# potsawee/tokenize-audio

Hardware: AMD Instinct MI355X
Metric: audio-sec encoded/sec (Mimi 8-codebook, 24 kHz) (higher is better)
Workload: dtype f16x3 (fp32-emulating: 2 fp16 planes per operand, 3 products, fp32 accumulate; RVQ distances fp32); 1 GPU; LibriTTS-R-style batch encode (configs[1]): batch=32 x 10 s @ 24 kHz resident in HBM, K=8 codebooks, 1 encode per step per GPU; global_batch=32, num_quantizers=8, parallelism=utterance round-robin x1 (no collective), gemm_precision=f16x3

## Files before the change

### tokenize-audio_amd/csrc/engine.cpp

```cpp
#include <hip/hip_runtime.h>

#include <algorithm>
#include <cmath>
#include <cstdarg>
#include <cstdio>
#include <cstdlib>
#include <cstring>
#include <fstream>
#include <map>
#include <memory>
#include <mutex>
#include <string>
#include <tuple>
#include <unordered_map>
#include <vector>

#include "../../include/mimi_hip.h"
#include "host_io.h"
#include "kernels.h"

using namespace mimi;

static thread_local std::string g_last_error;

// ... 267 lines not shown
    int stage0_fused = 1;
    int ln_fused = 1;
    int rvq_form = 0;
    int ln_rpw = 1;
    int rvq_xcd = 1;
    int rvq_chain = 1;
    bool chain_ok = false;
    unsigned* chain_flag = nullptr;
    int rvq_chain_fault = 0;
    int64_t chain_reruns = 0;
    int qkv_attn = 1;
    int qkv_attn_xcd = 1;
    int attn_band_split = 1;
    int sc1_out = 2;
    int fc1_cg = 1;
    int res1_form = 1;
    int res1_stream = 1;
    struct Tap {
        float* d = nullptr;
        size_t cap = 0;
        int64_t dims[3] = {0, 0, 0};
    };
    std::map<std::string, Tap> tapmap;

    bool decode_enabled = false;
    DevConv dec_first, dec_last;
    std::vector<DevConv> dec_up;
    std::vector<DevConv> dec_res3, dec_res1;
    std::vector<DevXfmr> dxf;
    float* outproj = nullptr;
// ... 1117 lines not shown
                ad.C = nullptr;
                xact = new_act("x_last");
                out_act(ad, xact);
            } else if (next_unf) {
                ad.Cp = w.xe;
                ad.c_pstride = (long long)B * p.T[si + 1] * 2 * C;
                role = ROLE_DOWN_XE;
                xeact = new_act(nmf("xe%d", si + 1));
                out_act(ad, xeact);
            }
        }
        if (rg) {
            ad.a_rows = dT[si];
            ad.m_rows = dT[si + 1];
        }
        LAUNCH_TRY(launch_gemm(role, ad, s, &kname, prec), "down");
        snprintf(nm, sizeof nm, "down_s%d", si);
        rec.mark(nm, gemm_flops(ad) * rows_of(si + 1, (double)B * p.T[si + 1]) / ((double)B * p.T[si + 1]),
                 gemm_bytes(ad, false), kname);
        snprintf(nm, sizeof nm, last ? "down%d_elu" : "down%d", si);
        if ((rc = save_tap_planes(e, nm, w.x, last ? ns : 0, B, p.T[si + 1], 2 * C, s, last ? xact.scale : 0.0f)))
            return rc;
        C *= 2;
    }
    const int64_t T = p.frames25;
    const int Hd = c.hidden_size;
    GemmArgs af = conv_args(e->final_conv, w.x, p.T[c.num_ratios], w.t0, T, B);
    if (ns) planes_in(af, w.x, (long long)B * p.T[c.num_ratios] * C);
    use_h(af, e->final_conv.wh, e->final_conv.wscale, xact);
    if (rg) {
        af.a_rows = dT[c.num_ratios];
// ... 14 lines not shown
        double f = 0;
        for (int64_t i = 0; i < Tn; ++i) f += 4.0 * Dh * std::min<int64_t>(i + 1, c.sliding_window);
        return f * H;
    };
    if (rg) {
        for (const auto& pb : rg->plan) att_flops += att_fl(pb.frames25);
    } else {
        att_flops = att_fl(T) * B;
    }
    for (int l = 0; l < c.num_hidden_layers; ++l) {
        const DevXfmr& x = e->xf[l];
        const long long nact = rows * Hd;
        Act t1a = new_act(nmf("xf%d.ln1", l));
        if (ln_check_free(t1a, x.ln1_bound)) t1a.amax = nullptr;
        auto ln_into = [&](GemmArgs& g, int role, const float* lw, const float* lb, const Act& act) {
            if (!h16 || e->ln_fused < (role == ROLE_QKV ? 2 : 1) || !gemm_ln_prologue_ok(role, g, prec)) return false;
            if (role == ROLE_QKV) g.ln_tile = e->ln_fused - 2;
            g.ln_x = w.t0;
            g.ln_g = lw;
            g.ln_b = lb;
            g.ln_eps = c.norm_eps;
            g.ln_scale = act.scale;
            g.ln_amax = act.amax;
            return true;
        };
        GemmArgs aq = linear_args(w.t1, T, Hd, x.wqkv, 3 * H * Dh, w.qkv);
        aq.Wsplit = x.wqkv_s;
        aq.batch = B;
        aq.a_bstride = T * Hd;
        aq.c_bstride = T * 3 * H * Dh;
        aq.rope_cos = e->rope_cos;
// ... 79 lines not shown
            use_h(a1, x.w1_h, x.w1_hs, t1b);
            a1.Cp = w.ff;
            a1.c_pstride = rows * c.intermediate_size;
            a1.C = nullptr;
            ffa = new_act(nmf("xf%d.ff", l));
            out_act(a1, ffa);
        }
        if (!ln_into(a1, ROLE_FC1, x.ln2_w, x.ln2_b, t1b)) {
            LAUNCH_TRY(launch_layernorm(w.t0, x.ln2_w, x.ln2_b, w.t1, rows, Hd, c.norm_eps, s, w.t1, nact, ns, t1b.scale,
                                        t1b.amax, nullptr, 0, e->ln_rpw),
                       "ln2");
            rec.mark("layernorm", 0, 2.0 * rows * Hd * 4, ln_kname(e->ln_rpw));
        }
        a1.sc1 = (e->sc1_out & 2) != 0;
        a1.ncg = e->fc1_cg;
        LAUNCH_TRY(launch_gemm(ROLE_FC1, a1, s, &kname, prec), "fc1");
        rec.mark("fc1", gemm_flops(a1), gemm_bytes(a1, false), kname);
        if ((rc = save_tap_planes(e, nmf("ff%d", l).c_str(), w.ff, ns, tapB, tapT, c.intermediate_size, s, ffa.scale)))
            return rc;
        GemmArgs a2 = linear_args(w.ff, rows, c.intermediate_size, x.w2, Hd, w.t0);
        a2.Wsplit = x.w2_s;
        a2.R = w.t0;
        a2.scale = x.ls2;
        if (ns) planes_in(a2, w.ff, rows * (long long)c.intermediate_size);
        use_h(a2, x.w2_h, x.w2_hs, ffa);
        if (ds_planes && l == c.num_hidden_layers - 1) {
            a2.Cp = w.t1;
            a2.c_pstride = nact;
            dsin = new_act("ds.in");
            out_act(a2, dsin);
        }
// ... 1219 lines not shown
    const char* values;
};
static const EngineOption kEngineOptions[] = {
    {"stage0_fused", &mimi_engine::stage0_fused, 0x3u, "0 or 1"},
    {"rvq_form", &mimi_engine::rvq_form, 0x7fu, "0..6"},
    {"ln_rpw", &mimi_engine::ln_rpw, 0x117u, "0, 1, 2, 4 or 8"},
    {"rvq_xcd", &mimi_engine::rvq_xcd, 0x3u, "0 or 1"},
    {"rvq_chain", &mimi_engine::rvq_chain, 0x3u, "0 or 1"},
    {"rvq_chain_fault", &mimi_engine::rvq_chain_fault, 0x7u, "0, 1 or 2"},
    {"sc1_out", &mimi_engine::sc1_out, 0xffu, "0..7"},
    {"ln_fused", &mimi_engine::ln_fused, 0x1fu, "0 .. 4"},
    {"qkv_attn", &mimi_engine::qkv_attn, 0x7u, "0, 1 or 2"},
    {"qkv_attn_xcd", &mimi_engine::qkv_attn_xcd, 0x3u, "0 or 1"},
    {"attn_band_split", &mimi_engine::attn_band_split, 0x7u, "0, 1 or 2"},
    {"fc1_cg", &mimi_engine::fc1_cg, 0x17u, "0, 1, 2 or 4"},
    {"res1_form", &mimi_engine::res1_form, 0x3u, "0 or 1"},
    {"res1_stream", &mimi_engine::res1_stream, 0x7u, "0, 1 or 2"},
};

extern "C" int mimi_set_option(mimi_engine* e, const char* key, int64_t value) {
    if (!e || !key) return set_err(MIMI_ERR_INVALID_ARGUMENT, "null engine or key");
    std::lock_guard<std::mutex> lk(e->mu);
    for (const EngineOption& o : kEngineOptions) {
        if (strcmp(key, o.key)) continue;
        if (value < 0 || value > 31 || !((o.allowed >> value) & 1u))
            return set_err(MIMI_ERR_INVALID_ARGUMENT, "%s %lld (%s)", key, (long long)value, o.values);
        HIP_TRY(hipSetDevice(e->device));
        if (e->*o.field != (int)value) {
            drop_graphs(e);
            e->graph_seen.clear();
// ... 156 lines not shown
```

### tokenize-audio_amd/csrc/gemm.hip

```cpp
#include <algorithm>
#include <cstdio>
#include <cstdlib>


#include "gemm_planes.h"

#ifndef MIMI_QKV_V
#define MIMI_QKV_V 1
#endif
#ifndef MIMI_FC1_V
#define MIMI_FC1_V 0
#endif
#ifndef MIMI_SMALL16_32W
#define MIMI_SMALL16_32W 1
#endif
#ifndef MIMI_SMALL16_32
#define MIMI_SMALL16_32 15
#endif


namespace mimi {

template <int BM, int BN, int WM, int WN, int BK, int NBUF, bool NFAST, bool ELU_IN, int PAD, int EPI, int TAG>
static const char* kernel_symbol() {
// ... 61 lines not shown
    long long grid = nwg;
    if (FL & FL_PERSIST) {
        static const int slots = [kern] {
            int dev = 0, ncu = 256, occ = 1;
            (void)hipGetDevice(&dev);
            (void)hipDeviceGetAttribute(&ncu, hipDeviceAttributeMultiprocessorCount, dev);
            (void)hipOccupancyMaxActiveBlocksPerMultiprocessor(&occ, kern, (WM * WN + LW) * 64, 0);
            return std::max(8, ncu * std::max(1, occ) / 8 * 8);
        }();
        grid = std::min<long long>(nwg, slots);
    }
    hipLaunchKernelGGL(kern, dim3((unsigned)grid), dim3((WM * WN + LW) * 64), 0, s, a);
    return hipGetLastError();
}

template <int EPI, int OUTP3, int OUTP2, int TAG>
static hipError_t run_planes_big(const GemmArgs& a, hipStream_t s, int prec) {
    if (prec == PREC_F16X3) return run_planes<256, 128, 4, 2, 2, 3, EPI, OUTP2, TAG, 0, 32, 16, 0, true>(a, s);
    if (prec == PREC_BF16X6) return run_planes<256, 128, 4, 2, 3, 2, EPI, OUTP3, TAG>(a, s);
    return run_planes<256, 128, 4, 2, 2, 3, EPI, OUTP2, TAG>(a, s);
}
template <int EPI, int OUTP3, int OUTP2, int TAG>
static hipError_t run_planes_big_ld(const GemmArgs& a, hipStream_t s, int prec) {
    if (prec == PREC_F16X3) return run_planes<256, 128, 4, 2, 2, 3, EPI, OUTP2, TAG, 0, 32, 16, 0, true>(a, s);
    if (prec == PREC_BF16X6) return run_planes<256, 128, 2, 2, 3, 2, EPI, OUTP3, TAG, 4>(a, s);
    return run_planes<256, 128, 2, 2, 2, 3, EPI, OUTP2, TAG, 4>(a, s);
}
template <int EPI, int TAG>
static hipError_t run_planes_small(const GemmArgs& a, hipStream_t s, int prec) {
    if (prec == PREC_F16X3) return run_planes<128, 128, 4, 2, 2, 4, EPI, 0, TAG, 0, 32, 16, 0, true>(a, s);
// ... 12 lines not shown

template <bool ELU_IN, int PAD, int EPI, int TAG>
static hipError_t run_prec(const GemmArgs& a, hipStream_t s, int prec);

template <bool ELU_IN, int PAD, int EPI, int TAG>
static hipError_t run_auto(const GemmArgs& a, hipStream_t s) {
    if (a.N <= 32) return run<256, 32, 4, 1, 32, 1, false, ELU_IN, PAD, EPI, TAG>(a, s);
    if (a.N <= 64) return run<256, 64, 4, 1, 32, 1, false, ELU_IN, PAD, EPI, TAG>(a, s);
    if (a.M <= 1024) return run<64, 128, 1, 2, 32, 1, false, ELU_IN, PAD, EPI, TAG>(a, s);
    return run<128, 128, 2, 2, 32, 1, false, ELU_IN, PAD, EPI, TAG>(a, s);
}

static hipError_t dispatch(int role, const GemmArgs& a, hipStream_t s);

static thread_local int g_prec = PREC_F32;

template <bool ELU_IN, int PAD, int EPI, int TAG>
static hipError_t run_prec(const GemmArgs& a, hipStream_t s, int prec) {
    if (prec == PREC_BF16X6 || prec == PREC_F16X3) return run_split<128, 128, 2, 2, 3, ELU_IN, PAD, EPI, TAG>(a, s);
    if (prec == PREC_BF16X3) return run_split<128, 128, 2, 2, 2, ELU_IN, PAD, EPI, TAG>(a, s);
    return run_auto<ELU_IN, PAD, EPI, TAG>(a, s);
}

__global__ __launch_bounds__(256) void gelu_check_kernel(const float* __restrict__ in, long long n,
                                                         float* __restrict__ out) {
    for (long long i = blockIdx.x * 256LL + threadIdx.x; i < n; i += (long long)gridDim.x * 256) out[i] = gelu_fast(in[i]);
}
hipError_t launch_gelu_check(const float* in, long long n, float* out, hipStream_t st) {
    if (n <= 0) return hipSuccess;
    const long long blocks = std::min<long long>((n + 255) / 256, 4096);
    hipLaunchKernelGGL(gelu_check_kernel, dim3((unsigned)blocks), dim3(256), 0, st, in, n, out);
    return hipGetLastError();
}

hipError_t launch_gemm(int role, const GemmArgs& a, hipStream_t s, const char** kname, int precision) {
    if (a.K % 32 != 0 || a.a_cin % 4 != 0 || a.a_rs % 4 != 0 || a.M <= 0 || a.N <= 0 || a.batch <= 0)
        return hipErrorInvalidValue;
    if (a.Ap && (a.a_cin % 8 != 0 || a.a_rs % 8 != 0 || a.a_off % 8 != 0)) return hipErrorInvalidValue;
    g_last_kernel = nullptr;
    g_prec = precision;
    hipError_t e = dispatch(role, a, s);
    if (kname) *kname = g_last_kernel ? g_last_kernel : "?";
    return e;
}

static bool pair_ok(const GemmArgs& a) {
    if (a.a_cin <= 0 || a.a_cin % 64 || a.K % a.a_cin || a.a_rs % a.a_cin) return false;
    const int k = a.K / a.a_cin, st = a.a_rs / a.a_cin;
    return st > 0 && k == 2 * st && a.K % 64 == 0;
}

constexpr long long kSmallGrid = 128;
static long long tiles(const GemmArgs& a, int bm, int bn) {
    return (long long)((a.M + bm - 1) / bm) * ((a.N + bn - 1) / bn) * a.batch;
}

#ifndef MIMI_DOWN_SMALL_ST
#define MIMI_DOWN_SMALL_ST 6
#endif
#ifndef MIMI_DOWN_SMALL2_ST
#define MIMI_DOWN_SMALL2_ST 3
#endif
template <int EPI, int OUTP, int TAG>
static hipError_t run_planes_down_h16(const GemmArgs& a, hipStream_t s) {
    if (pair_ok(a) && tiles(a, 256, 128) < kSmallGrid && a.K >= 4096) {
        if (tiles(a, 64, 64) < 256)
            return run_planes<32, 32, 1, 2, 2, MIMI_DOWN_SMALL_ST, EPI, OUTP, TAG, 4, 32, 16, FL_PAIR | FL_KG2, true>(a, s);
// ... 8 lines not shown

#ifndef MIMI_SMALL_ST
#define MIMI_SMALL_ST 4
#endif
#ifndef MIMI_LNA_ST
#define MIMI_LNA_ST 4
#endif
template <int EPI, int OUTP, int TAG, int BN0, int BM1, int BN1, int WM1, int WN1, int BN2, int WN2, int ST = MIMI_SMALL_ST,
          int FL = 0, int BM0 = 64, int WN0 = 2>
static hipError_t run_small_h16(const GemmArgs& a, hipStream_t s) {
    if (tiles(a, BM0, BN0) >= 256) return run_planes<BM0, BN0, 2, WN0, 2, ST, EPI, OUTP, TAG, 4, 32, 16, FL, true>(a, s);
    if (tiles(a, BM1, BN1) >= 256) return run_planes<BM1, BN1, WM1, WN1, 2, ST, EPI, OUTP, TAG, 4, 32, 16, FL, true>(a, s);
    return run_planes<16, BN2, 1, WN2, 2, ST, EPI, OUTP, TAG, 4, 32, 16, FL, true>(a, s);
}

bool gemm_ln_prologue_ok(int role, const GemmArgs& a, int precision) {
    return precision == PREC_F16X3 && (role == ROLE_QKV || role == ROLE_FC1) && a.K == 512 && a.a_rs == 512 &&
           a.a_off == 0 && !a.a_rows && !a.m_rows && !a.a_boff && tiles(a, 128, 128) < kSmallGrid;
}

static hipError_t dispatch_planes(int role, const GemmArgs& a, hipStream_t s) {
    const int prec = g_prec;
    if (prec != PREC_BF16X6 && prec != PREC_BF16X3 && prec != PREC_F16X3) return hipErrorInvalidValue;
    if (a.ln_x) {
        if (!gemm_ln_prologue_ok(role, a, prec) || !a.ln_g || !a.ln_b || !(a.ln_scale > 0.0f)) return hipErrorInvalidValue;
        if (role == ROLE_QKV) {
            if (tiles(a, 32, 128) >= 256) return run_planes<32, 128, 2, 2, 2, MIMI_LNA_ST, EPI_ROPE, 0, 5, 4, 32, 16, FL_LNA, true>(a, s);
            if (a.ln_tile == 1) return run_planes<32, 64, 2, 1, 2, MIMI_LNA_ST, EPI_ROPE, 0, 5, 4, 32, 16, FL_LNA, true>(a, s);
            if (a.ln_tile == 2) return run_planes<16, 128, 1, 2, 2, MIMI_LNA_ST, EPI_ROPE, 0, 5, 4, 32, 16, FL_LNA, true>(a, s);
            return run_planes<16, 64, 1, 1, 2, MIMI_LNA_ST, EPI_ROPE, 0, 5, 4, 32, 16, FL_LNA, true>(a, s);
        }
        if (tiles(a, 64, 64) >= 256) return run_planes<64, 64, 2, 2, 2, MIMI_LNA_ST, EPI_GELU, 2, 7, 4, 32, 16, FL_LNA, true>(a, s);
        if (tiles(a, 32, 64) >= 256) return run_planes<32, 64, 2, 2, 2, MIMI_LNA_ST, EPI_GELU, 2, 7, 4, 32, 16, FL_LNA, true>(a, s);
        return run_planes<16, 64, 1, 2, 2, MIMI_LNA_ST, EPI_GELU, 2, 7, 4, 32, 16, FL_LNA, true>(a, s);
    }
#ifndef MIMI_SMALL_ROLES
#define MIMI_SMALL_ROLES 1
#endif
    const bool qsmall = tiles(a, 128, 128) < 256 &&
                        (((MIMI_SMALL_ROLES & 1) && (role == ROLE_DOWNSAMPLE || role == ROLE_INPROJ)) ||
                         ((MIMI_SMALL_ROLES & 2) && role == ROLE_OPROJ) || ((MIMI_SMALL_ROLES & 4) && role == ROLE_FC2) ||
                         ((MIMI_SMALL_ROLES & 8) && role == ROLE_FINAL));
    if (prec == PREC_F16X3 && (tiles(a, 128, 128) < kSmallGrid || qsmall)) {
        switch (role) {
            case ROLE_FINAL:
                if (MIMI_SMALL16_32 & 2) return run_small_h16<EPI_BIAS_OUT, 0, 4, 64, 32, 64, 2, 2, 32, MIMI_SMALL16_32W>(a, s);
                return run_small_h16<EPI_BIAS_OUT, 0, 4, 64, 32, 64, 2, 2, 64, 2>(a, s);
            case ROLE_QKV: return run_small_h16<EPI_ROPE, 0, 5, 128, 32, 128, 2, 2, 64, 1>(a, s);
            case ROLE_OPROJ:
// ... 108 lines not shown
```

### tokenize-audio_amd/csrc/gemm_planes.h

```cpp
#pragma once
#include <type_traits>

#include "gemm_kernel.h"

namespace mimi {

#if defined(__HIP_DEVICE_COMPILE__)
__device__ __forceinline__ __amdgpu_buffer_rsrc_t make_rsrc(const void* base, long long bytes) {
    const long long lim = bytes < 0x7fffffffLL ? bytes : 0x7fffffffLL;
    return __builtin_amdgcn_make_buffer_rsrc(const_cast<void*>(base), (short)0, (int)lim, 0x00020000);
}
#endif

template <int PM, int L>
__device__ __forceinline__ void wait_stages(int later) {
    if constexpr (L == 0) {
        asm volatile("s_waitcnt vmcnt(0)" ::: "memory");
    } else {
        if (later >= L)
            asm volatile("s_waitcnt vmcnt(%0)" ::"n"(L * PM) : "memory");
        else
            wait_stages<PM, L - 1>(later);
    }
}
// ... 39 lines not shown
    constexpr int TPA = LNA ? 0 : NS * AR / RPP, TP = TPA + NS * NB * BN / RPP;
    constexpr int PMAX = (TP + NLD - 1) / NLD;
    constexpr int PMIN = TP / NLD;
    static_assert(BK == 32 || (BK == 16 && MF == 32), "BK");
    static_assert(MF == 32 || MF == 16, "MFMA shape");
    static_assert(TM >= 1 && TN >= 1 && KSUB >= 1, "tile");
    static_assert(NS * BM % RPP == 0 && NS * BN % RPP == 0, "whole pieces");
    static_assert(STAGES >= 2 * KG && STAGES <= 16, "stages");
    static_assert(PMAX * (STAGES - 2 * KG) <= 63, "vmcnt range");
    static_assert(EPI != EPI_ROPE || (MF == 32 ? TN % 2 == 0 : TN % 4 == 0), "rope pairs (d, d+32) in one lane");
    static_assert(!F16 || NS == 2, "fp16 planes: 2 planes, 3 products");
    static_assert(!LNA || (F16 && !PAIR && !(FL & (FL_PERSIST | FL_RAGGED | FL_DIAG_ILV))), "LayerNorm prologue");
    constexpr int LNK = 512;
    constexpr int LNE = LNA ? LNK / BK * NS * APL : 0;
    constexpr int ONS = OUTP & 7;
    constexpr bool OELU = (OUTP & 8) != 0;
    typedef typename std::conditional<MF == 32, f32x16, f32x4>::type accT;
    constexpr int NACC = MF == 32 ? 16 : 4;

    constexpr int CW = TN * MF, RW = TM * MF;
    constexpr int PFS0 = (STAGES - KG) * STG;
    constexpr bool PFIT1 = PFS0 * 2 + NW * RW * (CW + 4) * 4 <= 160 * 1024;
    constexpr bool PFIT2 = TN % 2 == 0 && PFS0 * 2 + NW * RW * (CW / 2 + 4) * 4 <= 160 * 1024;
    constexpr bool PFIT4 = TN % 4 == 0 && PFS0 * 2 + NW * RW * (CW / 4 + 4) * 4 <= 160 * 1024;
    constexpr bool PF = (FL & FL_PF) && (FL & FL_PERSIST) && LW > 0 && (PFIT1 || PFIT2 || PFIT4);
    constexpr int PFS = PF ? PFS0 : 0;
    constexpr int JH = PF ? (PFIT1 ? 1 : PFIT2 ? 2 : 4) : (NW * RW * (CW + 4) * 4 <= 160 * 1024 ? 1 : 2);
    constexpr int TNC = TN / JH, CWC = TNC * MF, LDE = CWC + 4;
    static_assert(TNC * JH == TN, "epilogue passes");
    constexpr int LDS_EL = STAGES * STG > PFS + NW * RW * LDE * 2 ? STAGES * STG : PFS + NW * RW * LDE * 2;
    static_assert((LDS_EL + LNE) * 2 <= 160 * 1024, "LDS");
// ... 379 lines not shown
#pragma unroll
            for (int img = 0; img < NB; ++img)
#pragma unroll
                for (int ks = 0; ks < KSUB; ++ks) {
                    read_frags(As, Bs, ks, af, bf, img);
                    if (!(FL & FL_DIAG_NOMMA)) mma_split<NS, TM, TN, F16>(acc, af, bf);
                }
        }
        if (FL & FL_PRIO) __builtin_amdgcn_s_setprio(0);
    }
    }

    __syncthreads();
    if (compute) {
    float* stg = reinterpret_cast<float*>(lds + PFS) + wave * (RW * LDE);
    const float* __restrict__ Rb = p.R ? p.R + c_base_of(b) : nullptr;
    const int rbase = m0 + wm * RW;
    const int cbase = n0 + wn * CW + (lane & (MF - 1));
    const float us = F16 ? p.unscale : 1.0f;
    const int Mb = RG ? min(M, p.m_rows[b]) : M;
#pragma unroll
    for (int jh = 0; jh < JH; ++jh) {
#pragma unroll
    for (int i = 0; i < TM; ++i) {
#pragma unroll
        for (int j = jh * TNC; j < (jh + 1) * TNC; ++j) {
            const int col = cbase + j * MF;
            float bias = 0.0f, scale = 0.0f;
            if (col < N) {
                if (EPI == EPI_BIAS || EPI == EPI_BIAS_ELU || EPI == EPI_BIAS_RES_ELU || EPI == EPI_BIAS_OUT)
                    bias = p.bias[col];
                if (EPI == EPI_SCALE_RES) scale = p.scale[col];
            }
#pragma unroll
            for (int r = 0; r < NACC; ++r) {
                const int lrow = MF == 32 ? i * 32 + (r & 3) + 8 * (r >> 2) + 4 * hsel : i * 16 + 4 * hsel + r;
                const int row = rbase + lrow;
                const bool ok = row < Mb && col < N;
                float v = F16 ? acc[i][j][r] * us : acc[i][j][r];
                if (EPI == EPI_BIAS || EPI == EPI_BIAS_OUT) {
                    v = v + bias;
                } else if (EPI == EPI_BIAS_ELU) {
                    v = elu1(v + bias);
                } else if (EPI == EPI_BIAS_RES_ELU) {
                    v = F16 ? __builtin_fmaf(acc[i][j][r], us, bias) : v + bias;
                } else if (EPI == EPI_GELU) {
                    v = F16 ? gelu_fast(v) : gelu_erf(v);
                } else if (EPI == EPI_SCALE_RES) {
                    v = scale * v;
                } else if (EPI == EPI_ROPE) {
                    if (ok && col < p.rope_cols) {
                        constexpr int PJ = 32 / MF;
                        const int d = col % 64;
                        const int pos = p.rope_pos ? p.rope_pos[row] : row;
                        const float c = p.rope_cos[(long long)pos * 32 + (d & 31)];
                        const float sn = p.rope_sin[(long long)pos * 32 + (d & 31)];
                        if (((j / PJ) & 1) == 0) {
                            const float x2 = F16 ? acc[i][j + PJ][r] * us : acc[i][j + PJ][r];
                            v = rope_lo(v, x2, c, sn);
                        } else {
                            const float x1 = F16 ? acc[i][j - PJ][r] * us : acc[i][j - PJ][r];
                            v = rope_hi(v, x1, c, sn);
                        }
                    }
                }
                stg[lrow * LDE + (j - jh * TNC) * MF + (lane & (MF - 1))] = v;
            }
        }
    }
    float* __restrict__ Cb = p.C ? p.C + c_base_of(b) : nullptr;
    static_assert(!F16 || ONS == 0 || ONS == 2, "fp16 output planes: 2");
    __bf16* __restrict__ Cpb = ONS ? reinterpret_cast<__bf16*>(p.Cp) + c_base_of(b) : nullptr;
    constexpr bool SC1 = (FL & FL_SC1OUT) != 0;
    static_assert(!SC1 || !ONS || F16, "sc1 output stores: fp32 and fp16 planes");
    typedef unsigned u32x4 __attribute__((ext_vector_type(4)));
    const __amdgpu_buffer_rsrc_t c_rs = make_rsrc(SC1 ? (void*)Cb : nullptr, SC1 ? 0x7fffffffLL : 0);
    const __amdgpu_buffer_rsrc_t cp_rs = make_rsrc(SC1 ? (void*)Cpb : nullptr, SC1 ? 0x7fffffffLL : 0);
    constexpr int LPR = CWC / 8;
    constexpr int RPS = 64 / LPR;
    static_assert(RW % RPS == 0 || RW < RPS, "epilogue: a wave's tile holds whole passes of 64 lanes x 8 columns");
    constexpr int NPS = RW < RPS ? 1 : RW / RPS;
#pragma unroll
    for (int ps = 0; ps < NPS; ++ps) {
        const int lr = ps * RPS + lane / LPR, lc = (lane % LPR) * 8;
        if (RW < RPS && lr >= RW) continue;
        f32x4 v0 = *reinterpret_cast<const f32x4*>(stg + lr * LDE + lc);
        f32x4 v1 = *reinterpret_cast<const f32x4*>(stg + lr * LDE + lc + 4);
        const int row = m0 + wm * RW + lr, col = n0 + wn * CW + jh * CWC + lc;
        if (row >= Mb || col >= N) continue;
        const long long off = (long long)row * p.ldc + col;
        if (EPI == EPI_BIAS_RES_ELU || EPI == EPI_SCALE_RES) {
            const f32x4 r0 = *reinterpret_cast<const f32x4*>(Rb + off);
            const f32x4 r1 = *reinterpret_cast<const f32x4*>(Rb + off + 4);
            v0 = r0 + v0;
            v1 = r1 + v1;
            if (EPI == EPI_BIAS_RES_ELU) {
                v0.x = elu1(v0.x); v0.y = elu1(v0.y); v0.z = elu1(v0.z); v0.w = elu1(v0.w);
                v1.x = elu1(v1.x); v1.y = elu1(v1.y); v1.z = elu1(v1.z); v1.w = elu1(v1.w);
            }
        }
        if (ONS) {
            float pv[8] = {v0.x, v0.y, v0.z, v0.w, v1.x, v1.y, v1.z, v1.w};
            if (OELU) {
#pragma unroll
                for (int e = 0; e < 8; ++e) pv[e] = elu1(pv[e]);
            }
            if constexpr (SC1) {
                uint4 ha, hb;
                split2_f16s(pv[0], pv[1], p.out_scale, ha.x, hb.x);
                split2_f16s(pv[2], pv[3], p.out_scale, ha.y, hb.y);
                split2_f16s(pv[4], pv[5], p.out_scale, ha.z, hb.z);
                split2_f16s(pv[6], pv[7], p.out_scale, ha.w, hb.w);
#pragma unroll
                for (int e = 0; e < 8; ++e) omx = fmaxf(omx, fabsf(pv[e]));
                __builtin_amdgcn_raw_buffer_store_b128(__builtin_bit_cast(u32x4, ha), cp_rs, (int)(off * 2), 0, 16);
                __builtin_amdgcn_raw_buffer_store_b128(__builtin_bit_cast(u32x4, hb), cp_rs,
                                                       (int)((off + p.c_pstride) * 2), 0, 16);
            } else {
                store_act8(Cpb, p.c_pstride, ONS, off, pv, F16 ? p.out_scale : 0.0f, &omx);
            }
        }
        if (Cb) {
            if constexpr (SC1) {
                __builtin_amdgcn_raw_buffer_store_b128(__builtin_bit_cast(u32x4, v0), c_rs, (int)(off * 4), 0, 16);
                __builtin_amdgcn_raw_buffer_store_b128(__builtin_bit_cast(u32x4, v1), c_rs, (int)(off * 4 + 16), 0, 16);
            } else {
                *reinterpret_cast<f32x4*>(Cb + off) = v0;
                *reinterpret_cast<f32x4*>(Cb + off + 4) = v1;
            }
        }
    }
    asm volatile("" ::: "memory");
    }
    }
    if (FL & FL_PERSIST) {
        asm volatile("s_waitcnt lgkmcnt(0)" ::: "memory");
        __builtin_amdgcn_s_barrier();
    }
    }
    if (F16 && ONS && compute) amax_commit(p.out_amax, omx);
    if (LNA && compute) amax_commit(p.ln_amax, ln_mx);
#endif
}

}
```

### tokenize-audio_amd/csrc/kernels.h

```cpp
#pragma once
#include <hip/hip_runtime.h>
#include <cstdint>

namespace mimi {

int set_error_message(int code, const char* msg);

__device__ __forceinline__ float elu_fast(float x) {
    const float e = __expf(x) - 1.0f;
    return x > 0.0f ? x : e;
}

__device__ __forceinline__ void store_act(float* f32, void* planes, long long pstride, int ns, long long idx,
                                          float v, float hscale = 0.0f, float* mx = nullptr) {
    if (ns == 0) {
        f32[idx] = v;
        return;
    }
    if (hscale > 0.0f) {
        _Float16* hp = reinterpret_cast<_Float16*>(planes) + idx;
        const float t = v * hscale;
        const _Float16 h0 = (_Float16)t;
        hp[0] = h0;
        hp[pstride] = (_Float16)(t - (float)h0);
// ... 152 lines not shown
    const int* a_boff;
    const int* c_boff;
    const int* rope_pos;
    const float* ln_x;
    const float* ln_g;
    const float* ln_b;
    float ln_eps;
    float ln_scale;
    unsigned* ln_amax;
    int sc1;
    int ln_tile;
    int ncg;
};
bool res1_stream_ok(const GemmArgs& a);
hipError_t launch_res1_stream(const GemmArgs& a, hipStream_t s, const char** kname);
bool gemm_ln_prologue_ok(int role, const GemmArgs& a, int precision);

enum GemmRole : int {
    ROLE_RES3 = 0,
    ROLE_RES1,
    ROLE_DOWN,
    ROLE_DOWN_ELU,
    ROLE_FINAL,
    ROLE_QKV,
    ROLE_OPROJ,
    ROLE_FC1,
    ROLE_FC2,
    ROLE_DOWNSAMPLE,
    ROLE_INPROJ,
    ROLE_DOWN_XE,
    ROLE_RES3P,
    ROLE_RES1P,
    ROLE_UPCONV,
    ROLE_COUNT
};
enum Precision : int { PREC_F32 = 0, PREC_BF16X6 = 1, PREC_BF16X3 = 2, PREC_F16X3 = 3 };

hipError_t launch_gemm(int role, const GemmArgs& a, hipStream_t s, const char** kname = nullptr,
                       int precision = PREC_F32);

struct ResArgs {
    const float* x;
    const float* audio;
    const float* const* audio_ref;
    const float* w0;
    const float* b0;
    long long T;
    int batch;
    const float* w3;
    const float* b3;
    const float* w1;
    const float* b1;
    float* y;
    void* yp;
// ... 116 lines not shown
```

Measured before the change: 52110 audio-sec/sec.

## Add 256x256-tile 8-wave f16x3 GEMM kernel for FC1 and downsample convs

Adds a new 512-thread GEMM kernel with 256x256 output tiles, an 8-stage LDS ring and split early/late wave phases. It is used for FC1 and the downsampling convolution GEMMs when the grid holds enough 256x256 tiles, and the down convs can run persistently. The shared epilogue is moved into an include file so both kernels use it. Larger tiles raise operand reuse and arithmetic intensity, at the cost of fewer workgroups, higher register and LDS pressure, and only firing on large shapes outside the ragged-batch path.

```diff
diff --git a/tokenize-audio_amd/csrc/engine.cpp b/tokenize-audio_amd/csrc/engine.cpp
--- a/tokenize-audio_amd/csrc/engine.cpp
+++ b/tokenize-audio_amd/csrc/engine.cpp
@@ -305,6 +305,7 @@
     int attn_band_split = 1;
     int sc1_out = 2;
     int fc1_cg = 1;
+    int gemm256 = 3;
     int res1_form = 1;
     int res1_stream = 1;
     struct Tap {
@@ -1452,7 +1453,7 @@
             ad.a_rows = dT[si];
             ad.m_rows = dT[si + 1];
         }
-        LAUNCH_TRY(launch_gemm(role, ad, s, &kname, prec), "down");
+        LAUNCH_TRY(launch_gemm(role, ad, s, &kname, prec, rg ? 0 : e->gemm256), "down");
         snprintf(nm, sizeof nm, "down_s%d", si);
         rec.mark(nm, gemm_flops(ad) * rows_of(si + 1, (double)B * p.T[si + 1]) / ((double)B * p.T[si + 1]),
                  gemm_bytes(ad, false), kname);
@@ -1497,7 +1498,7 @@
         Act t1a = new_act(nmf("xf%d.ln1", l));
         if (ln_check_free(t1a, x.ln1_bound)) t1a.amax = nullptr;
         auto ln_into = [&](GemmArgs& g, int role, const float* lw, const float* lb, const Act& act) {
-            if (!h16 || e->ln_fused < (role == ROLE_QKV ? 2 : 1) || !gemm_ln_prologue_ok(role, g, prec)) return false;
+            if (!h16 || e->ln_fused < (role == ROLE_QKV ? 2 : 1) || !gemm_ln_prologue_ok(role, g, prec, rg ? 0 : e->gemm256)) return false;
             if (role == ROLE_QKV) g.ln_tile = e->ln_fused - 2;
             g.ln_x = w.t0;
             g.ln_g = lw;
@@ -1607,7 +1608,7 @@
         }
         a1.sc1 = (e->sc1_out & 2) != 0;
         a1.ncg = e->fc1_cg;
-        LAUNCH_TRY(launch_gemm(ROLE_FC1, a1, s, &kname, prec), "fc1");
+        LAUNCH_TRY(launch_gemm(ROLE_FC1, a1, s, &kname, prec, rg ? 0 : e->gemm256), "fc1");
         rec.mark("fc1", gemm_flops(a1), gemm_bytes(a1, false), kname);
         if ((rc = save_tap_planes(e, nmf("ff%d", l).c_str(), w.ff, ns, tapB, tapT, c.intermediate_size, s, ffa.scale)))
             return rc;
@@ -2857,6 +2858,7 @@
     {"qkv_attn_xcd", &mimi_engine::qkv_attn_xcd, 0x3u, "0 or 1"},
     {"attn_band_split", &mimi_engine::attn_band_split, 0x7u, "0, 1 or 2"},
     {"fc1_cg", &mimi_engine::fc1_cg, 0x17u, "0, 1, 2 or 4"},
+    {"gemm256", &mimi_engine::gemm256, 0xffu, "0..7"},
     {"res1_form", &mimi_engine::res1_form, 0x3u, "0 or 1"},
     {"res1_stream", &mimi_engine::res1_stream, 0x7u, "0, 1 or 2"},
 };
diff --git a/tokenize-audio_amd/csrc/gemm.hip b/tokenize-audio_amd/csrc/gemm.hip
--- a/tokenize-audio_amd/csrc/gemm.hip
+++ b/tokenize-audio_amd/csrc/gemm.hip
@@ -4,6 +4,7 @@
 
 
 #include "gemm_planes.h"
+#include "gemm_planes256.h"
 
 #ifndef MIMI_QKV_V
 #define MIMI_QKV_V 1
@@ -99,6 +100,43 @@
     return hipGetLastError();
 }
 
+static bool pair_ok(const GemmArgs& a);
+static long long tiles(const GemmArgs& a, int bm, int bn);
+
+static bool planes256_ok(const GemmArgs& a) {
+    return a.Ap && a.Wsplit && !a.ln_x && !a.m_rows && !a.a_rows && !a.a_boff && !a.c_boff && !a.R && a.K % 32 == 0 &&
+           a.K >= 64 && 2LL * a.N * a.K < 0x7fffffffLL && a.a_len * 2 <= 0x7fffffffLL && a.N % 8 == 0 && a.ldc % 8 == 0 &&
+           a.c_bstride % 8 == 0 && a.c_pstride % 8 == 0;
+}
+template <int EPI, int OUTP, int TAG, int FL>
+static hipError_t run_planes256(const GemmArgs& a, hipStream_t s) {
+    static thread_local char name[96];
+    if (!name[0]) snprintf(name, sizeof(name), "mimi::gemm_planes256_kernel<%d, %d, %d, %d>", EPI, OUTP, TAG, FL);
+    g_last_kernel = name;
+    if (!planes256_ok(a) || ((OUTP & 7) && (!a.Cp || a.out_scale <= 0.0f)) || (!(OUTP & 7) && !a.C) || ((OUTP & 8) && !a.C))
+        return hipErrorInvalidValue;
+    if ((FL & FL_PAIR) && !pair_ok(a)) return hipErrorInvalidValue;
+    const long long nwg = tiles(a, 256, 256);
+    if (nwg > 0x7fffffffLL) return hipErrorInvalidValue;
+    if constexpr ((FL & FL_SC1OUT) != 0) {
+        const long long rows = a.M;
+        if ((rows * a.ldc + a.N) * 4 > 0x7fffffffLL || ((OUTP & 7) && (a.c_pstride + rows * a.ldc) * 2 > 0x7fffffffLL))
+            return run_planes256<EPI, OUTP, TAG, FL & ~FL_SC1OUT>(a, s);
+    }
+    long long grid = nwg;
+    if (FL & FL_PERSIST) {
+        static const int slots = [] {
+            int dev = 0, ncu = 256;
+            (void)hipGetDevice(&dev);
+            (void)hipDeviceGetAttribute(&ncu, hipDeviceAttributeMultiprocessorCount, dev);
+            return std::max(8, ncu / 8 * 8);
+        }();
+        grid = std::min<long long>(nwg, slots);
+    }
+    hipLaunchKernelGGL((gemm_planes256_kernel<EPI, OUTP, TAG, FL>), dim3((unsigned)grid), dim3(512), 0, s, a);
+    return hipGetLastError();
+}
+
 template <int EPI, int OUTP3, int OUTP2, int TAG>
 static hipError_t run_planes_big(const GemmArgs& a, hipStream_t s, int prec) {
     if (prec == PREC_F16X3) return run_planes<256, 128, 4, 2, 2, 3, EPI, OUTP2, TAG, 0, 32, 16, 0, true>(a, s);
@@ -141,6 +179,7 @@
 static hipError_t dispatch(int role, const GemmArgs& a, hipStream_t s);
 
 static thread_local int g_prec = PREC_F32;
+static thread_local int g_g256 = 0;
 
 template <bool ELU_IN, int PAD, int EPI, int TAG>
 static hipError_t run_prec(const GemmArgs& a, hipStream_t s, int prec) {
@@ -160,12 +199,13 @@
     return hipGetLastError();
 }
 
-hipError_t launch_gemm(int role, const GemmArgs& a, hipStream_t s, const char** kname, int precision) {
+hipError_t launch_gemm(int role, const GemmArgs& a, hipStream_t s, const char** kname, int precision, int g256) {
     if (a.K % 32 != 0 || a.a_cin % 4 != 0 || a.a_rs % 4 != 0 || a.M <= 0 || a.N <= 0 || a.batch <= 0)
         return hipErrorInvalidValue;
     if (a.Ap && (a.a_cin % 8 != 0 || a.a_rs % 8 != 0 || a.a_off % 8 != 0)) return hipErrorInvalidValue;
     g_last_kernel = nullptr;
     g_prec = precision;
+    g_g256 = g256;
     hipError_t e = dispatch(role, a, s);
     if (kname) *kname = g_last_kernel ? g_last_kernel : "?";
     return e;
@@ -178,6 +218,7 @@
 }
 
 constexpr long long kSmallGrid = 128;
+constexpr long long kGrid256 = 256;
 static long long tiles(const GemmArgs& a, int bm, int bn) {
     return (long long)((a.M + bm - 1) / bm) * ((a.N + bn - 1) / bn) * a.batch;
 }
@@ -216,7 +257,8 @@
     return run_planes<16, BN2, 1, WN2, 2, ST, EPI, OUTP, TAG, 4, 32, 16, FL, true>(a, s);
 }
 
-bool gemm_ln_prologue_ok(int role, const GemmArgs& a, int precision) {
+bool gemm_ln_prologue_ok(int role, const GemmArgs& a, int precision, int g256) {
+    if (role == ROLE_FC1 && (g256 & 4)) return false;
     return precision == PREC_F16X3 && (role == ROLE_QKV || role == ROLE_FC1) && a.K == 512 && a.a_rs == 512 &&
            a.a_off == 0 && !a.a_rows && !a.m_rows && !a.a_boff && tiles(a, 128, 128) < kSmallGrid;
 }
@@ -235,6 +277,18 @@
         if (tiles(a, 64, 64) >= 256) return run_planes<64, 64, 2, 2, 2, MIMI_LNA_ST, EPI_GELU, 2, 7, 4, 32, 16, FL_LNA, true>(a, s);
         if (tiles(a, 32, 64) >= 256) return run_planes<32, 64, 2, 2, 2, MIMI_LNA_ST, EPI_GELU, 2, 7, 4, 32, 16, FL_LNA, true>(a, s);
         return run_planes<16, 64, 1, 2, 2, MIMI_LNA_ST, EPI_GELU, 2, 7, 4, 32, 16, FL_LNA, true>(a, s);
+    }
+    if (prec == PREC_F16X3 && g_g256 && planes256_ok(a)) {
+        const bool force = (g_g256 & 4) != 0;
+        const bool grid_ok = force || (tiles(a, 256, 256) >= kGrid256 && a.N >= 256);
+        if (role == ROLE_FC1 && (force || (g_g256 & 1)) && grid_ok && a.Cp) {
+            if (a.sc1) return run_planes256<EPI_GELU, 2, 7, FL_SC1OUT>(a, s);
+            return run_planes256<EPI_GELU, 2, 7, 0>(a, s);
+        }
+        if ((role == ROLE_DOWN || role == ROLE_DOWN_XE) && (force || (g_g256 & 2)) && grid_ok && pair_ok(a)) {
+            if (role == ROLE_DOWN) return run_planes256<EPI_BIAS, 0, 2, FL_PAIR | FL_PERSIST>(a, s);
+            return run_planes256<EPI_BIAS, 2 | 8, 11, FL_PAIR | FL_PERSIST>(a, s);
+        }
     }
 #ifndef MIMI_SMALL_ROLES
 #define MIMI_SMALL_ROLES 1
diff --git a/tokenize-audio_amd/csrc/gemm_planes.h b/tokenize-audio_amd/csrc/gemm_planes.h
--- a/tokenize-audio_amd/csrc/gemm_planes.h
+++ b/tokenize-audio_amd/csrc/gemm_planes.h
@@ -77,7 +77,6 @@
     constexpr int LNK = 512;
     constexpr int LNE = LNA ? LNK / BK * NS * APL : 0;
     constexpr int ONS = OUTP & 7;
-    constexpr bool OELU = (OUTP & 8) != 0;
     typedef typename std::conditional<MF == 32, f32x16, f32x4>::type accT;
     constexpr int NACC = MF == 32 ? 16 : 4;
 
@@ -487,124 +486,10 @@
     __syncthreads();
     if (compute) {
     float* stg = reinterpret_cast<float*>(lds + PFS) + wave * (RW * LDE);
-    const float* __restrict__ Rb = p.R ? p.R + c_base_of(b) : nullptr;
-    const int rbase = m0 + wm * RW;
-    const int cbase = n0 + wn * CW + (lane & (MF - 1));
-    const float us = F16 ? p.unscale : 1.0f;
+    const long long cel = c_base_of(b);
+    const int rbase = m0 + wm * RW, cb0 = n0 + wn * CW;
     const int Mb = RG ? min(M, p.m_rows[b]) : M;
-#pragma unroll
-    for (int jh = 0; jh < JH; ++jh) {
-#pragma unroll
-    for (int i = 0; i < TM; ++i) {
-#pragma unroll
-        for (int j = jh * TNC; j < (jh + 1) * TNC; ++j) {
-            const int col = cbase + j * MF;
-            float bias = 0.0f, scale = 0.0f;
-            if (col < N) {
-                if (EPI == EPI_BIAS || EPI == EPI_BIAS_ELU || EPI == EPI_BIAS_RES_ELU || EPI == EPI_BIAS_OUT)
-                    bias = p.bias[col];
-                if (EPI == EPI_SCALE_RES) scale = p.scale[col];
-            }
-#pragma unroll
-            for (int r = 0; r < NACC; ++r) {
-                const int lrow = MF == 32 ? i * 32 + (r & 3) + 8 * (r >> 2) + 4 * hsel : i * 16 + 4 * hsel + r;
-                const int row = rbase + lrow;
-                const bool ok = row < Mb && col < N;
-                float v = F16 ? acc[i][j][r] * us : acc[i][j][r];
-                if (EPI == EPI_BIAS || EPI == EPI_BIAS_OUT) {
-                    v = v + bias;
-                } else if (EPI == EPI_BIAS_ELU) {
-                    v = elu1(v + bias);
-                } else if (EPI == EPI_BIAS_RES_ELU) {
-                    v = F16 ? __builtin_fmaf(acc[i][j][r], us, bias) : v + bias;
-                } else if (EPI == EPI_GELU) {
-                    v = F16 ? gelu_fast(v) : gelu_erf(v);
-                } else if (EPI == EPI_SCALE_RES) {
-                    v = scale * v;
-                } else if (EPI == EPI_ROPE) {
-                    if (ok && col < p.rope_cols) {
-                        constexpr int PJ = 32 / MF;
-                        const int d = col % 64;
-                        const int pos = p.rope_pos ? p.rope_pos[row] : row;
-                        const float c = p.rope_cos[(long long)pos * 32 + (d & 31)];
-                        const float sn = p.rope_sin[(long long)pos * 32 + (d & 31)];
-                        if (((j / PJ) & 1) == 0) {
-                            const float x2 = F16 ? acc[i][j + PJ][r] * us : acc[i][j + PJ][r];
-                            v = rope_lo(v, x2, c, sn);
-                        } else {
-                            const float x1 = F16 ? acc[i][j - PJ][r] * us : acc[i][j - PJ][r];
-                            v = rope_hi(v, x1, c, sn);
-                        }
-                    }
-                }
-                stg[lrow * LDE + (j - jh * TNC) * MF + (lane & (MF - 1))] = v;
-            }
-        }
-    }
-    float* __restrict__ Cb = p.C ? p.C + c_base_of(b) : nullptr;
-    static_assert(!F16 || ONS == 0 || ONS == 2, "fp16 output planes: 2");
-    __bf16* __restrict__ Cpb = ONS ? reinterpret_cast<__bf16*>(p.Cp) + c_base_of(b) : nullptr;
-    constexpr bool SC1 = (FL & FL_SC1OUT) != 0;
-    static_assert(!SC1 || !ONS || F16, "sc1 output stores: fp32 and fp16 planes");
-    typedef unsigned u32x4 __attribute__((ext_vector_type(4)));
-    const __amdgpu_buffer_rsrc_t c_rs = make_rsrc(SC1 ? (void*)Cb : nullptr, SC1 ? 0x7fffffffLL : 0);
-    const __amdgpu_buffer_rsrc_t cp_rs = make_rsrc(SC1 ? (void*)Cpb : nullptr, SC1 ? 0x7fffffffLL : 0);
-    constexpr int LPR = CWC / 8;
-    constexpr int RPS = 64 / LPR;
-    static_assert(RW % RPS == 0 || RW < RPS, "epilogue: a wave's tile holds whole passes of 64 lanes x 8 columns");
-    constexpr int NPS = RW < RPS ? 1 : RW / RPS;
-#pragma unroll
-    for (int ps = 0; ps < NPS; ++ps) {
-        const int lr = ps * RPS + lane / LPR, lc = (lane % LPR) * 8;
-        if (RW < RPS && lr >= RW) continue;
-        f32x4 v0 = *reinterpret_cast<const f32x4*>(stg + lr * LDE + lc);
-        f32x4 v1 = *reinterpret_cast<const f32x4*>(stg + lr * LDE + lc + 4);
-        const int row = m0 + wm * RW + lr, col = n0 + wn * CW + jh * CWC + lc;
-        if (row >= Mb || col >= N) continue;
-        const long long off = (long long)row * p.ldc + col;
-        if (EPI == EPI_BIAS_RES_ELU || EPI == EPI_SCALE_RES) {
-            const f32x4 r0 = *reinterpret_cast<const f32x4*>(Rb + off);
-            const f32x4 r1 = *reinterpret_cast<const f32x4*>(Rb + off + 4);
-            v0 = r0 + v0;
-            v1 = r1 + v1;
-            if (EPI == EPI_BIAS_RES_ELU) {
-                v0.x = elu1(v0.x); v0.y = elu1(v0.y); v0.z = elu1(v0.z); v0.w = elu1(v0.w);
-                v1.x = elu1(v1.x); v1.y = elu1(v1.y); v1.z = elu1(v1.z); v1.w = elu1(v1.w);
-            }
-        }
-        if (ONS) {
-            float pv[8] = {v0.x, v0.y, v0.z, v0.w, v1.x, v1.y, v1.z, v1.w};
-            if (OELU) {
-#pragma unroll
-                for (int e = 0; e < 8; ++e) pv[e] = elu1(pv[e]);
-            }
-            if constexpr (SC1) {
-                uint4 ha, hb;
-                split2_f16s(pv[0], pv[1], p.out_scale, ha.x, hb.x);
-                split2_f16s(pv[2], pv[3], p.out_scale, ha.y, hb.y);
-                split2_f16s(pv[4], pv[5], p.out_scale, ha.z, hb.z);
-                split2_f16s(pv[6], pv[7], p.out_scale, ha.w, hb.w);
-#pragma unroll
-                for (int e = 0; e < 8; ++e) omx = fmaxf(omx, fabsf(pv[e]));
-                __builtin_amdgcn_raw_buffer_store_b128(__builtin_bit_cast(u32x4, ha), cp_rs, (int)(off * 2), 0, 16);
-                __builtin_amdgcn_raw_buffer_store_b128(__builtin_bit_cast(u32x4, hb), cp_rs,
-                                                       (int)((off + p.c_pstride) * 2), 0, 16);
-            } else {
-                store_act8(Cpb, p.c_pstride, ONS, off, pv, F16 ? p.out_scale : 0.0f, &omx);
-            }
-        }
-        if (Cb) {
-            if constexpr (SC1) {
-                __builtin_amdgcn_raw_buffer_store_b128(__builtin_bit_cast(u32x4, v0), c_rs, (int)(off * 4), 0, 16);
-                __builtin_amdgcn_raw_buffer_store_b128(__builtin_bit_cast(u32x4, v1), c_rs, (int)(off * 4 + 16), 0, 16);
-            } else {
-                *reinterpret_cast<f32x4*>(Cb + off) = v0;
-                *reinterpret_cast<f32x4*>(Cb + off + 4) = v1;
-            }
-        }
-    }
-    asm volatile("" ::: "memory");
-    }
+#include "gemm_planes_epilogue.inc"
     }
     if (FL & FL_PERSIST) {
         asm volatile("s_waitcnt lgkmcnt(0)" ::: "memory");
diff --git a/tokenize-audio_amd/csrc/gemm_planes256.h b/tokenize-audio_amd/csrc/gemm_planes256.h
--- /dev/null
+++ b/tokenize-audio_amd/csrc/gemm_planes256.h
@@ -0,0 +1,215 @@
+#pragma once
+#include "gemm_planes.h"
+
+namespace mimi {
+
+template <int EPI, int OUTP, int TAG, int FL = 0>
+__global__ __launch_bounds__(512) void gemm_planes256_kernel(GemmArgs p) {
+#if defined(__HIP_DEVICE_COMPILE__)
+    constexpr int BM = 256, BN = 256, BK = 32, MF = 16, NW = 8;
+    constexpr int TM = 8, TN = 4;
+    constexpr int PL = 128 * BK;
+    constexpr int HT = 2 * PL;
+    constexpr int RING = 8 * HT;
+    constexpr bool PAIR = (FL & FL_PAIR) != 0;
+    constexpr int ONS = OUTP & 7;
+    constexpr int JH = 2, LDE = TN * MF / JH + 4;
+    constexpr int LDS_EL = RING > NW * TM * MF * LDE * 2 ? RING : NW * TM * MF * LDE * 2;
+    static_assert(LDS_EL * 2 <= 160 * 1024, "LDS");
+    __shared__ __attribute__((aligned(16))) __bf16 lds[LDS_EL];
+
+    const int tid = threadIdx.x;
+    const int lane = tid & 63;
+    const int wave = __builtin_amdgcn_readfirstlane(tid >> 6);
+    const int wm = wave >> 2, wn = wave & 3;
+    const bool late = wave >= 4;
+    const int M = p.M, N = p.N, K = p.K;
+    const int MT = (M + BM - 1) / BM, NTn = (N + BN - 1) / BN;
+    const int ntiles = MT * NTn * p.batch;
+    const int KT = K / BK;
+    const int NH = 4 * KT;
+    const int ncg = (p.ncg > 1 && NTn % p.ncg == 0) ? p.ncg : 1;
+    float omx = 0.0f;
+
+    const int prow = wave * 16 + (lane >> 2), pch = lane & 3;
+    const int csrc = (pch ^ chunk_swz<BK, MF>(prow)) * 8;
+    const int a_trow = (prow >> 6) * 128 + (prow & 63);
+    const int b_tcol = (prow >> 5) * 64 + (prow & 31);
+    const __bf16* __restrict__ Wp = reinterpret_cast<const __bf16*>(p.Wsplit);
+    const int w_pl = N * K;
+
+    const int fr = lane & 15, hsel = lane >> 4;
+    const int a_frag = (wm * 64 + fr) * BK + ((hsel ^ chunk_swz<BK, MF>(fr)) * 8);
+    const int b_frag = (wn * 32 + fr) * BK + ((hsel ^ chunk_swz<BK, MF>(fr)) * 8);
+
+    for (int tile = blockIdx.x; tile < ntiles; tile += gridDim.x) {
+    int b, mt, nt;
+    {
+        const int logical = xcd_remap(tile, ntiles);
+        int rest;
+        if (ncg > 1) {
+            const int NG = NTn / ncg, per = ntiles / ncg;
+            const int cg = logical / per, w = logical - cg * per;
+            nt = cg * NG + w % NG;
+            rest = w / NG;
+        } else {
+            nt = logical % NTn;
+            rest = logical / NTn;
+        }
+        mt = __builtin_amdgcn_readfirstlane(rest % MT);
+        b = __builtin_amdgcn_readfirstlane(rest / MT);
+        nt = __builtin_amdgcn_readfirstlane(nt);
+    }
+    const int m0 = mt * BM, n0 = nt * BN;
+    const __bf16* __restrict__ Abase = reinterpret_cast<const __bf16*>(p.Ap) + (long long)b * p.a_bstride;
+    const __amdgpu_buffer_rsrc_t ars0 = make_rsrc(Abase, p.a_len * 2);
+    const __amdgpu_buffer_rsrc_t ars1 = make_rsrc(Abase + p.a_pstride, p.a_len * 2);
+    int a_src[2], b_src[2];
+#pragma unroll
+    for (int h = 0; h < 2; ++h) {
+        const int m = m0 + a_trow + h * 64;
+        a_src[h] = m < M ? (int)((p.a_off + (long long)m * p.a_rs + csrc) * 2) : -16;
+        int n = n0 + b_tcol + h * 32;
+        n = n < N ? n : N - 1;
+        b_src[h] = n * K + csrc;
+    }
+
+    KOrderT<BK> ko;
+    ko.init(p, PAIR);
+    const int ktap = PAIR ? ko.s * ko.cin : 0;
+    int kstep = 0;
+    auto k_of_issue = [&]() {
+        return PAIR ? ko.offset() + (kstep & 1) * ktap : ko.offset();
+    };
+    auto k_advance = [&]() {
+        if (!PAIR || (kstep & 1)) ko.next();
+        ++kstep;
+    };
+    auto issue = [&](int slot, auto rc, int k0) {
+        constexpr int r = decltype(rc)::value;
+        __bf16* dst = lds + (slot * 4 + r) * HT + wave * 16 * BK;
+        if constexpr (r & 1) {
+            const int off = a_src[r >> 1] + k0 * 2;
+            __builtin_amdgcn_raw_ptr_buffer_load_lds(ars0, (__attribute__((address_space(3))) void*)dst, 16, off, 0, 0, 0);
+            __builtin_amdgcn_raw_ptr_buffer_load_lds(ars1, (__attribute__((address_space(3))) void*)(dst + PL), 16, off,
+                                                     0, 0, 0);
+        } else {
+            const __bf16* src = Wp + b_src[r >> 1] + k0;
+            __builtin_amdgcn_global_load_lds((const void*)src, (__attribute__((address_space(3))) void*)dst, 16, 0, 0);
+            __builtin_amdgcn_global_load_lds((const void*)(src + w_pl), (__attribute__((address_space(3))) void*)(dst + PL),
+                                             16, 0, 0);
+        }
+    };
+
+    f32x4 acc[TM][TN];
+#pragma unroll
+    for (int i = 0; i < TM; ++i)
+#pragma unroll
+        for (int j = 0; j < TN; ++j)
+#pragma unroll
+            for (int r = 0; r < 4; ++r) acc[i][j][r] = 0.0f;
+
+    {
+        const int k0 = k_of_issue();
+        k_advance();
+        issue(0, std::integral_constant<int, 0>(), k0);
+        issue(0, std::integral_constant<int, 1>(), k0);
+        issue(0, std::integral_constant<int, 2>(), k0);
+        issue(0, std::integral_constant<int, 3>(), k0);
+    }
+    int kiss = k_of_issue();
+    k_advance();
+    issue(1, std::integral_constant<int, 0>(), kiss);
+    issue(1, std::integral_constant<int, 1>(), kiss);
+    asm volatile("s_waitcnt vmcnt(8)" ::: "memory");
+    __builtin_amdgcn_s_barrier();
+    if (late) __builtin_amdgcn_s_barrier();
+    asm volatile("" ::: "memory");
+
+    bf16x8 af[2][4], bf[2][2][2];
+    auto read_a = [&](const __bf16* ht) {
+#pragma unroll
+        for (int pl = 0; pl < 2; ++pl)
+#pragma unroll
+            for (int i = 0; i < 4; ++i) af[pl][i] = *reinterpret_cast<const bf16x8*>(ht + pl * PL + a_frag + i * 16 * BK);
+    };
+    auto read_b = [&](const __bf16* ht, int sb) {
+#pragma unroll
+        for (int pl = 0; pl < 2; ++pl)
+#pragma unroll
+            for (int j = 0; j < 2; ++j) bf[sb][pl][j] = *reinterpret_cast<const bf16x8*>(ht + pl * PL + b_frag + j * 16 * BK);
+    };
+    auto mma_quad = [&](auto sac, auto sbc) {
+        constexpr int sa = decltype(sac)::value, sb = decltype(sbc)::value;
+        if (FL & FL_DIAG_NOMMA) return;
+#pragma unroll
+        for (int i = 0; i < 4; ++i)
+#pragma unroll
+            for (int j = 0; j < 2; ++j) {
+                f32x4& c = acc[sa * 4 + i][sb * 2 + j];
+                c = mfma16<true>(af[1][i], bf[sb][0][j], c);
+                c = mfma16<true>(af[0][i], bf[sb][1][j], c);
+                c = mfma16<true>(af[0][i], bf[sb][0][j], c);
+            }
+    };
+    auto phase_tail = [&](int pphase, int slot_iss, auto rc, auto sac, auto sbc) {
+        const int h = pphase + 6;
+        if (!(FL & FL_DIAG_NODMA) && h < NH) issue(slot_iss, rc, kiss);
+        wait_stages<2, 4>(min(4, max(0, NH - 3 - pphase)));
+        __builtin_amdgcn_s_barrier();
+        asm volatile("s_waitcnt lgkmcnt(0)" ::: "memory");
+        __builtin_amdgcn_sched_barrier(0);
+        __builtin_amdgcn_s_setprio(1);
+        mma_quad(sac, sbc);
+        __builtin_amdgcn_s_setprio(0);
+        __builtin_amdgcn_sched_barrier(0);
+        __builtin_amdgcn_s_barrier();
+        asm volatile("" ::: "memory");
+    };
+    using I0 = std::integral_constant<int, 0>;
+    using I1 = std::integral_constant<int, 1>;
+    using I2 = std::integral_constant<int, 2>;
+    using I3 = std::integral_constant<int, 3>;
+
+    for (int kt = 0; kt < KT; ++kt) {
+        const __bf16* st = lds + (kt & 1) * 4 * HT;
+        const int s1 = (kt + 1) & 1, s2 = kt & 1;
+        const int p0 = 4 * kt;
+        read_b(st + 0 * HT, 0);
+        __builtin_amdgcn_sched_barrier(0);
+        read_a(st + 1 * HT);
+        asm volatile("" ::: "memory");
+        phase_tail(p0 + 0, s1, I2(), I0(), I0());
+        read_b(st + 2 * HT, 1);
+        asm volatile("" ::: "memory");
+        phase_tail(p0 + 1, s1, I3(), I0(), I1());
+        read_a(st + 3 * HT);
+        asm volatile("" ::: "memory");
+        if (kt + 2 < KT) {
+            kiss = k_of_issue();
+            k_advance();
+        }
+        phase_tail(p0 + 2, s2, I0(), I1(), I1());
+        phase_tail(p0 + 3, s2, I1(), I1(), I0());
+    }
+    if (!late) __builtin_amdgcn_s_barrier();
+
+    __syncthreads();
+    {
+    constexpr bool F16 = true;
+    float* stg = reinterpret_cast<float*>(lds) + wave * (TM * MF * LDE);
+    const long long cel = (long long)b * p.c_bstride;
+    const int rbase = m0 + wm * TM * MF, cb0 = n0 + wn * TN * MF;
+    const int Mb = M;
+#include "gemm_planes_epilogue.inc"
+    }
+    if (FL & FL_PERSIST) {
+        asm volatile("s_waitcnt lgkmcnt(0)" ::: "memory");
+        __builtin_amdgcn_s_barrier();
+    }
+    }
+    if (ONS) amax_commit(p.out_amax, omx);
+#endif
+}
+
+}
diff --git a/tokenize-audio_amd/csrc/gemm_planes_epilogue.inc b/tokenize-audio_amd/csrc/gemm_planes_epilogue.inc
--- /dev/null
+++ b/tokenize-audio_amd/csrc/gemm_planes_epilogue.inc
@@ -0,0 +1,124 @@
+{
+    constexpr int ONS = OUTP & 7;
+    constexpr bool OELU = (OUTP & 8) != 0;
+    constexpr int NACC = MF == 32 ? 16 : 4;
+    constexpr int RW = TM * MF, TNC = TN / JH, CWC = TNC * MF, LDE = CWC + 4;
+    const int N = p.N;
+    const int hsel = MF == 32 ? lane >> 5 : lane >> 4;
+    const float* __restrict__ Rb = p.R ? p.R + cel : nullptr;
+    const int cbase = cb0 + (lane & (MF - 1));
+    const float us = F16 ? p.unscale : 1.0f;
+#pragma unroll
+    for (int jh = 0; jh < JH; ++jh) {
+#pragma unroll
+    for (int i = 0; i < TM; ++i) {
+#pragma unroll
+        for (int j = jh * TNC; j < (jh + 1) * TNC; ++j) {
+            const int col = cbase + j * MF;
+            float bias = 0.0f, scale = 0.0f;
+            if (col < N) {
+                if (EPI == EPI_BIAS || EPI == EPI_BIAS_ELU || EPI == EPI_BIAS_RES_ELU || EPI == EPI_BIAS_OUT)
+                    bias = p.bias[col];
+                if (EPI == EPI_SCALE_RES) scale = p.scale[col];
+            }
+#pragma unroll
+            for (int r = 0; r < NACC; ++r) {
+                const int lrow = MF == 32 ? i * 32 + (r & 3) + 8 * (r >> 2) + 4 * hsel : i * 16 + 4 * hsel + r;
+                const int row = rbase + lrow;
+                const bool ok = row < Mb && col < N;
+                float v = F16 ? acc[i][j][r] * us : acc[i][j][r];
+                if (EPI == EPI_BIAS || EPI == EPI_BIAS_OUT) {
+                    v = v + bias;
+                } else if (EPI == EPI_BIAS_ELU) {
+                    v = elu1(v + bias);
+                } else if (EPI == EPI_BIAS_RES_ELU) {
+                    v = F16 ? __builtin_fmaf(acc[i][j][r], us, bias) : v + bias;
+                } else if (EPI == EPI_GELU) {
+                    v = F16 ? gelu_fast(v) : gelu_erf(v);
+                } else if (EPI == EPI_SCALE_RES) {
+                    v = scale * v;
+                } else if (EPI == EPI_ROPE) {
+                    if (ok && col < p.rope_cols) {
+                        constexpr int PJ = 32 / MF;
+                        const int d = col % 64;
+                        const int pos = p.rope_pos ? p.rope_pos[row] : row;
+                        const float c = p.rope_cos[(long long)pos * 32 + (d & 31)];
+                        const float sn = p.rope_sin[(long long)pos * 32 + (d & 31)];
+                        if (((j / PJ) & 1) == 0) {
+                            const float x2 = F16 ? acc[i][j + PJ][r] * us : acc[i][j + PJ][r];
+                            v = rope_lo(v, x2, c, sn);
+                        } else {
+                            const float x1 = F16 ? acc[i][j - PJ][r] * us : acc[i][j - PJ][r];
+                            v = rope_hi(v, x1, c, sn);
+                        }
+                    }
+                }
+                stg[lrow * LDE + (j - jh * TNC) * MF + (lane & (MF - 1))] = v;
+            }
+        }
+    }
+    float* __restrict__ Cb = p.C ? p.C + cel : nullptr;
+    static_assert(!F16 || ONS == 0 || ONS == 2, "fp16 output planes: 2");
+    __bf16* __restrict__ Cpb = ONS ? reinterpret_cast<__bf16*>(p.Cp) + cel : nullptr;
+    constexpr bool SC1 = (FL & FL_SC1OUT) != 0;
+    static_assert(!SC1 || !ONS || F16, "sc1 output stores: fp32 and fp16 planes");
+    typedef unsigned u32x4 __attribute__((ext_vector_type(4)));
+    const __amdgpu_buffer_rsrc_t c_rs = make_rsrc(SC1 ? (void*)Cb : nullptr, SC1 ? 0x7fffffffLL : 0);
+    const __amdgpu_buffer_rsrc_t cp_rs = make_rsrc(SC1 ? (void*)Cpb : nullptr, SC1 ? 0x7fffffffLL : 0);
+    constexpr int LPR = CWC / 8;
+    constexpr int RPS = 64 / LPR;
+    static_assert(RW % RPS == 0 || RW < RPS, "epilogue: a wave's tile holds whole passes of 64 lanes x 8 columns");
+    constexpr int NPS = RW < RPS ? 1 : RW / RPS;
+#pragma unroll
+    for (int ps = 0; ps < NPS; ++ps) {
+        const int lr = ps * RPS + lane / LPR, lc = (lane % LPR) * 8;
+        if (RW < RPS && lr >= RW) continue;
+        f32x4 v0 = *reinterpret_cast<const f32x4*>(stg + lr * LDE + lc);
+        f32x4 v1 = *reinterpret_cast<const f32x4*>(stg + lr * LDE + lc + 4);
+        const int row = rbase + lr, col = cb0 + jh * CWC + lc;
+        if (row >= Mb || col >= N) continue;
+        const long long off = (long long)row * p.ldc + col;
+        if (EPI == EPI_BIAS_RES_ELU || EPI == EPI_SCALE_RES) {
+            const f32x4 r0 = *reinterpret_cast<const f32x4*>(Rb + off);
+            const f32x4 r1 = *reinterpret_cast<const f32x4*>(Rb + off + 4);
+            v0 = r0 + v0;
+            v1 = r1 + v1;
+            if (EPI == EPI_BIAS_RES_ELU) {
+                v0.x = elu1(v0.x); v0.y = elu1(v0.y); v0.z = elu1(v0.z); v0.w = elu1(v0.w);
+                v1.x = elu1(v1.x); v1.y = elu1(v1.y); v1.z = elu1(v1.z); v1.w = elu1(v1.w);
+            }
+        }
+        if (ONS) {
+            float pv[8] = {v0.x, v0.y, v0.z, v0.w, v1.x, v1.y, v1.z, v1.w};
+            if (OELU) {
+#pragma unroll
+                for (int e = 0; e < 8; ++e) pv[e] = elu1(pv[e]);
+            }
+            if constexpr (SC1) {
+                uint4 ha, hb;
+                split2_f16s(pv[0], pv[1], p.out_scale, ha.x, hb.x);
+                split2_f16s(pv[2], pv[3], p.out_scale, ha.y, hb.y);
+                split2_f16s(pv[4], pv[5], p.out_scale, ha.z, hb.z);
+                split2_f16s(pv[6], pv[7], p.out_scale, ha.w, hb.w);
+#pragma unroll
+                for (int e = 0; e < 8; ++e) omx = fmaxf(omx, fabsf(pv[e]));
+                __builtin_amdgcn_raw_buffer_store_b128(__builtin_bit_cast(u32x4, ha), cp_rs, (int)(off * 2), 0, 16);
+                __builtin_amdgcn_raw_buffer_store_b128(__builtin_bit_cast(u32x4, hb), cp_rs,
+                                                       (int)((off + p.c_pstride) * 2), 0, 16);
+            } else {
+                store_act8(Cpb, p.c_pstride, ONS, off, pv, F16 ? p.out_scale : 0.0f, &omx);
+            }
+        }
+        if (Cb) {
+            if constexpr (SC1) {
+                __builtin_amdgcn_raw_buffer_store_b128(__builtin_bit_cast(u32x4, v0), c_rs, (int)(off * 4), 0, 16);
+                __builtin_amdgcn_raw_buffer_store_b128(__builtin_bit_cast(u32x4, v1), c_rs, (int)(off * 4 + 16), 0, 16);
+            } else {
+                *reinterpret_cast<f32x4*>(Cb + off) = v0;
+                *reinterpret_cast<f32x4*>(Cb + off + 4) = v1;
+            }
+        }
+    }
+    asm volatile("" ::: "memory");
+    }
+}
diff --git a/tokenize-audio_amd/csrc/kernels.h b/tokenize-audio_amd/csrc/kernels.h
--- a/tokenize-audio_amd/csrc/kernels.h
+++ b/tokenize-audio_amd/csrc/kernels.h
@@ -190,7 +190,7 @@
 };
 bool res1_stream_ok(const GemmArgs& a);
 hipError_t launch_res1_stream(const GemmArgs& a, hipStream_t s, const char** kname);
-bool gemm_ln_prologue_ok(int role, const GemmArgs& a, int precision);
+bool gemm_ln_prologue_ok(int role, const GemmArgs& a, int precision, int g256 = 0);
 
 enum GemmRole : int {
     ROLE_RES3 = 0,
@@ -213,7 +213,7 @@
 enum Precision : int { PREC_F32 = 0, PREC_BF16X6 = 1, PREC_BF16X3 = 2, PREC_F16X3 = 3 };
 
 hipError_t launch_gemm(int role, const GemmArgs& a, hipStream_t s, const char** kname = nullptr,
-                       int precision = PREC_F32);
+                       int precision = PREC_F32, int g256 = 0);
 
 struct ResArgs {
     const float* x;
```

New measurement: 53320 audio-sec/sec, median of 6. 1.02x the previous value.
